# VaibhavKamat/Performance-Comparison-of-TensorFlow-PyTorch-and-their-Distributed-Counterparts

Hardware: AMD Instinct MI355X
Metric: resnet50_train_images_per_sec (higher is better)
Workload: dtype bf16; 1 GPU; model=resnet50, global_batch=256, per_gpu_batch=256, image_size=224, num_classes=1000, parallelism=dp1, impl=hip, optimizer=sgd_momentum, hipgraph=False, ddp_force=False, grad_allreduce_dtype=fp32, lr_warmup_steps=5

## Files before the change

### performance-comparison-of-tensorflow-pytorch-and-their-distributed-counterparts_amd/csrc/bnr_stream.h

```cpp
#pragma once
#include "igemm.h"

namespace pcmp {

inline Knob kn_bnr_stream("bnr_stream", 1);
inline Knob kn_bnr_stream_wgs("bnr_stream_wgs", 256);

template <int BN, int GK, bool FOLD, bool DUAL>
__global__ void __launch_bounds__(256, 2) bnr_stream_kernel(const IgemmParams p, int groups) {
  constexpr int BM = 32, NTHR = 256;
  constexpr int KB = GK / 64;
  constexpr int A_IMG = BM * GK * 2;
  constexpr int STAGE = A_IMG * (FOLD ? 2 : 1);
  constexpr int W_BYTES = BN * GK * 2;
  constexpr int CS = BN + 8;
  constexpr int C_BYTES = BM * CS * 4;
  constexpr int CPR = BN / 8;
  constexpr int NCH = BM * BN / 8 / NTHR;
  constexpr int RPP = NTHR / CPR;
  constexpr int NS = DUAL ? 3 : 2;
  constexpr int NWT = BN / 32;
  constexpr int NAI = A_IMG / 1024 / 4;
  constexpr int NWI = W_BYTES / 1024 / 4;
  constexpr int NEL = NCH * (DUAL ? 4 : 3);
  static_assert(NCH >= 1 && NAI >= 1 && NWI >= 1 && NWT <= 4, "bnr_stream tile");
  extern __shared__ __attribute__((aligned(16))) char smem[];
  char* sW = smem;
  char* sS = smem + W_BYTES;
  float* sC = reinterpret_cast<float*>(smem + W_BYTES + 2 * STAGE);
  float* sK = sC + BM * CS;

  const int tid = threadIdx.x, lane = tid & 63;
  const int wid = __builtin_amdgcn_readfirstlane(tid >> 6);
  const int ntn = p.gn / BN;
  const int lin = xcd_remap(blockIdx.x, gridDim.x);
  const int grp = lin / ntn, n0 = (lin - grp * ntn) * BN;
  const int npt = p.gm / BM;
  const int nmine = grp < npt ? (npt - 1 - grp) / groups + 1 : 0;

  const __amdgpu_buffer_rsrc_t rsA = make_rsrc(p.a, p.a_bytes);
  const __amdgpu_buffer_rsrc_t rsF = make_rsrc(FOLD ? p.fold_x : p.a, p.a_bytes);
  const __amdgpu_buffer_rsrc_t rsW = make_rsrc(p.b, p.b_bytes);
  const unsigned ebytes = (unsigned)((size_t)p.gm * p.gn * 2);
  const bool has_res = p.resid != nullptr;
  const unsigned rbytes = !has_res ? 0u : (p.resid_sub ? (unsigned)((size_t)p.N * p.rs_H2 * p.rs_W2 * p.gn * 2) : ebytes);
  const __amdgpu_buffer_rsrc_t rsR = make_rsrc(has_res ? (const void*)p.resid : (const void*)p.a, rbytes);
  const __amdgpu_buffer_rsrc_t rsX = make_rsrc(p.bn_x, ebytes);
  const __amdgpu_buffer_rsrc_t rsX2 = make_rsrc(DUAL ? p.bn_x2 : p.bn_x, DUAL ? ebytes : 0u);
  const bool has_mb = p.bn_mbits != nullptr;
  const __amdgpu_buffer_rsrc_t rsM = make_rsrc(has_mb ? (const void*)p.bn_mbits : (const void*)p.a,
                                               has_mb ? (unsigned)((size_t)p.gm * p.gn / 8) : 0u);

  const int lch = (lane & 7) ^ ((lane >> 3) & 7);
  int a_vo[NAI];
#pragma unroll
  for (int i = 0; i < NAI; ++i) {
    const int u = wid * NAI + i;
    const int row = (u & 3) * 8 + (lane >> 3);
    a_vo[i] = (row * GK + (u >> 2) * 64 + lch * 8) * 2;
  }
  const __amdgpu_buffer_rsrc_t rsZ = make_rsrc(p.a, 0u);
  auto issue_a = [&](int s, int pt, bool live) {
    char* dst = sS + s * STAGE;
    const int so = live ? pt * BM * GK * 2 : 0;
    const __amdgpu_buffer_rsrc_t ra = live ? rsA : rsZ, rf = live ? rsF : rsZ;
#pragma unroll
    for (int i = 0; i < NAI; ++i) {
      const int vo = a_vo[i];
      __builtin_amdgcn_raw_ptr_buffer_load_lds(ra, (__attribute__((address_space(3))) void*)(dst + (wid * NAI + i) * 1024),
                                               16, vo, so, 0, 0);
    }
    if constexpr (FOLD) {
#pragma unroll
      for (int i = 0; i < NAI; ++i) {
        const int vo = a_vo[i];
        __builtin_amdgcn_raw_ptr_buffer_load_lds(
            rf, (__attribute__((address_space(3))) void*)(dst + A_IMG + (wid * NAI + i) * 1024), 16, vo, so, 0, 0);
      }
    }
  };

  const int c8 = tid % CPR, r0 = tid / CPR;
  uint4 eR[2][NCH], eX[2][NCH], eX2[2][DUAL ? NCH : 1];
  unsigned eM[2][NCH];
  auto issue_e = [&](auto sel, int pt, bool live) {
    constexpr int E = decltype(sel)::value;
    if (!live) pt = 0;
    unsigned o[NCH], ro[NCH];
#pragma unroll
    for (int k = 0; k < NCH; ++k) {
      const int m = pt * BM + r0 + k * RPP;
      o[k] = (unsigned)m * (unsigned)p.gn + (unsigned)(n0 + c8 * 8);
      ro[k] = o[k] * 2u;
      if (p.resid_sub) {
        const unsigned n = fdiv((unsigned)m, p.fd_HW);
        const unsigned rem = (unsigned)m - n * (unsigned)(p.H * p.W);
        const unsigned hh = fdiv(rem, p.fd_W);
        const unsigned ww = rem - hh * (unsigned)p.W;
        ro[k] = ((hh | ww) & 1u) ? kOOB
                                 : (((n * (unsigned)p.rs_H2 + (hh >> 1)) * (unsigned)p.rs_W2 + (ww >> 1)) * (unsigned)p.gn +
                                    (unsigned)(n0 + c8 * 8)) * 2u;
      }
    }
#pragma unroll
    for (int k = 0; k < NCH; ++k) {
      if (!live) { o[k] = kOOB / 2u; ro[k] = kOOB; }
    }
#pragma unroll
    for (int k = 0; k < NCH; ++k) {
      eR[E][k] = bload16(rsR, ro[k]);
      eX[E][k] = bload16(rsX, o[k] * 2u);
      if constexpr (DUAL) eX2[E][k] = bload16(rsX2, o[k] * 2u);
      eM[E][k] = __builtin_amdgcn_raw_buffer_load_b32(rsM, (int)((o[k] >> 3) & ~3u), 0, 0);
    }
  };

  float ka[8], kb[8], ka2[DUAL ? 8 : 1], kb2[DUAL ? 8 : 1], msc[8], msh[8];
  const bool mfx = !has_mb;
#pragma unroll
  for (int e = 0; e < 8; ++e) {
    const int c = n0 + c8 * 8 + e;
    const float is = p.bn_istd[c];
    ka[e] = is;
    kb[e] = -p.bn_mean[c] * is;
    msc[e] = mfx ? p.bn_msc[c] : 0.f;
    msh[e] = mfx ? p.bn_msh[c] : 0.f;
    if constexpr (DUAL) {
      const float is2 = p.bn_istd2[c];
      ka2[e] = is2;
      kb2[e] = -p.bn_mean2[c] * is2;
    }
  }
  float sm[NS][8];
#pragma unroll
  for (int q = 0; q < NS; ++q)
#pragma unroll
    for (int e = 0; e < 8; ++e) sm[q][e] = 0.f;

  {
    int w_vo[NWI];
#pragma unroll
    for (int i = 0; i < NWI; ++i) {
      const int u = wid * NWI + i;
      const int row = (u % (BN / 8)) * 8 + (lane >> 3);
      w_vo[i] = ((n0 + row) * GK + (u / (BN / 8)) * 64 + lch * 8) * 2;
    }
#pragma unroll
    for (int i = 0; i < NWI; ++i) {
      const int vo = w_vo[i];
      __builtin_amdgcn_raw_ptr_buffer_load_lds(rsW, (__attribute__((address_space(3))) void*)(sW + (wid * NWI + i) * 1024),
                                               16, vo, 0, 0, 0);
    }
  }
  if constexpr (FOLD) {
    for (int i = tid; i < 3 * GK; i += NTHR) sK[i] = p.fold_coef[(i / GK) * p.K + (i % GK)];
  }
  const int pt0 = grp;
  issue_a(0, pt0, nmine > 0);
  issue_e(std::integral_constant<int, 0>{}, pt0, nmine > 0);
  wait_vm_b<0>();
  lds_sync_b();

  auto tile = [&](auto sel, int j) {
    constexpr int S = decltype(sel)::value;
    const int pt = pt0 + j * groups;
    if (j > 0) {
      wait_vm_b<NEL + NCH>();
      lds_sync_b();
    }
    char* sA = sS + S * STAGE;
    if constexpr (FOLD) {
#pragma unroll
      for (int i = 0; i < KB; ++i) {
        const int row = tid >> 3;
        const int kc = i * 64 + (((tid & 7) ^ (row & 7)) << 3);
        char* gp = sA + i * (BM * 128) + tid * 16;
        const uint4 g = *reinterpret_cast<const uint4*>(gp);
        const uint4 x = *reinterpret_cast<const uint4*>(gp + A_IMG);
        float k1[8], k2[8], k3[8];
#pragma unroll
        for (int h = 0; h < 2; ++h) {
          const f32x4 a = *reinterpret_cast<const f32x4*>(sK + kc + 4 * h);
          const f32x4 b = *reinterpret_cast<const f32x4*>(sK + GK + kc + 4 * h);
          const f32x4 c = *reinterpret_cast<const f32x4*>(sK + 2 * GK + kc + 4 * h);
#pragma unroll
          for (int e = 0; e < 4; ++e) { k1[4 * h + e] = a[e]; k2[4 * h + e] = b[e]; k3[4 * h + e] = c[e]; }
        }
        *reinterpret_cast<uint4*>(gp) = fold_dz(g, x, k1, k2, k3, true);
      }
      lds_sync_b();
    }
    __builtin_amdgcn_sched_barrier(0);
    const bool more = j + 1 < nmine;
    issue_a(S ^ 1, pt + groups, more);
    __builtin_amdgcn_sched_barrier(0);
    issue_e(std::integral_constant<int, S ^ 1>{}, pt + groups, more);
    __builtin_amdgcn_sched_barrier(0);
    if (wid < NWT) {
      f32x16 acc;
#pragma unroll
      for (int r = 0; r < 16; ++r) acc[r] = 0.f;
#pragma unroll
      for (int ks = 0; ks < GK / 16; ++ks) {
        const int ch = ks * 2 + (lane >> 5);
        const int kb = ch >> 3, cc = ch & 7;
        const bf16x8 fa = *reinterpret_cast<const bf16x8*>(sA + kb * (BM * 128) + rr_off(lane & 31, cc));
        const bf16x8 fb = *reinterpret_cast<const bf16x8*>(sW + kb * (BN * 128) + rr_off(wid * 32 + (lane & 31), cc));
        acc = __builtin_amdgcn_mfma_f32_32x32x16_bf16(fa, fb, acc, 0, 0, 0);
      }
#pragma unroll
      for (int r = 0; r < 16; ++r)
        sC[(8 * (r >> 2) + 4 * (lane >> 5) + (r & 3)) * CS + wid * 32 + (lane & 31)] = acc[r];
    }
    lds_sync_b();
    __bf16* out = reinterpret_cast<__bf16*>(p.out);
    const int mshift = ((n0 + c8 * 8) >> 3 & 3) * 8;
#pragma unroll
    for (int k = 0; k < NCH; ++k) {
      const int row = r0 + k * RPP;
      const f32x4 a0 = *reinterpret_cast<const f32x4*>(sC + row * CS + c8 * 8);
      const f32x4 a1 = *reinterpret_cast<const f32x4*>(sC + row * CS + c8 * 8 + 4);
      const float av[8] = {a0[0], a0[1], a0[2], a0[3], a1[0], a1[1], a1[2], a1[3]};
      const unsigned rw[4] = {eR[S][k].x, eR[S][k].y, eR[S][k].z, eR[S][k].w};
      const unsigned xw[4] = {eX[S][k].x, eX[S][k].y, eX[S][k].z, eX[S][k].w};
      unsigned ov[4];
#pragma unroll
      for (int q = 0; q < 4; ++q) {
        const float x0 = av[2 * q] + __uint_as_float(rw[q] << 16);
        const float x1 = av[2 * q + 1] + __uint_as_float(rw[q] & 0xffff0000u);
        unsigned u = f2bf2(x0, x1);
        const float xa = __uint_as_float(xw[q] << 16), xb = __uint_as_float(xw[q] & 0xffff0000u);
        const float z0 = fmaf(xa, msc[2 * q], msh[2 * q]);
        const float z1 = fmaf(xb, msc[2 * q + 1], msh[2 * q + 1]);
        const unsigned kz = (z0 > 0.f ? 0x0000ffffu : 0u) | (z1 > 0.f ? 0xffff0000u : 0u);
        const unsigned bits = eM[S][k] >> (mshift + 2 * q);
        const unsigned kbits = ((bits & 1u) ? 0x0000ffffu : 0u) | ((bits & 2u) ? 0xffff0000u : 0u);
        u &= mfx ? kz : kbits;
        const float g0 = __uint_as_float(u << 16), g1 = __uint_as_float(u & 0xffff0000u);
        sm[0][2 * q] += g0;
        sm[0][2 * q + 1] += g1;
        sm[1][2 * q] += g0 * fmaf(xa, ka[2 * q], kb[2 * q]);
        sm[1][2 * q + 1] += g1 * fmaf(xb, ka[2 * q + 1], kb[2 * q + 1]);
        if constexpr (DUAL) {
          const unsigned x2w = q == 0 ? eX2[S][k].x : q == 1 ? eX2[S][k].y : q == 2 ? eX2[S][k].z : eX2[S][k].w;
          sm[2][2 * q] += g0 * fmaf(__uint_as_float(x2w << 16), ka2[2 * q], kb2[2 * q]);
          sm[2][2 * q + 1] += g1 * fmaf(__uint_as_float(x2w & 0xffff0000u), ka2[2 * q + 1], kb2[2 * q + 1]);
        }
        ov[q] = u;
      }
      const size_t o = (size_t)(pt * BM + row) * p.gn + n0 + c8 * 8;
      *reinterpret_cast<uint4*>(out + o) = uint4{ov[0], ov[1], ov[2], ov[3]};
    }
  };
  int j = 0;
  for (; j + 1 < nmine; j += 2) {
    tile(std::integral_constant<int, 0>{}, j);
    tile(std::integral_constant<int, 1>{}, j + 1);
  }
  if (j < nmine) tile(std::integral_constant<int, 0>{}, j);

  __syncthreads();
  float* red = reinterpret_cast<float*>(sS);
#pragma unroll
  for (int q = 0; q < NS; ++q) {
    *reinterpret_cast<f32x4*>(red + (r0 * NS + q) * BN + c8 * 8) = f32x4{sm[q][0], sm[q][1], sm[q][2], sm[q][3]};
    *reinterpret_cast<f32x4*>(red + (r0 * NS + q) * BN + c8 * 8 + 4) = f32x4{sm[q][4], sm[q][5], sm[q][6], sm[q][7]};
  }
  __syncthreads();
  for (int i = tid; i < NS * BN; i += NTHR) {
    const int q = i / BN, c = i - q * BN;
    float t = 0.f;
    for (int r = 0; r < RPP; ++r) t += red[(r * NS + q) * BN + c];
    float* st = p.stats + (size_t)grp * 2 * p.gn;
    if (q == 0) {
      st[n0 + c] = t;
      if constexpr (DUAL) p.stats2[(size_t)grp * 2 * p.gn + n0 + c] = t;
    } else if (q == 1) {
      st[p.gn + n0 + c] = t;
    } else {
      p.stats2[(size_t)grp * 2 * p.gn + p.gn + n0 + c] = t;
    }
  }
}

static int bnr_stream_bn(const IgemmParams& p) { return p.gn == 64 ? 64 : 128; }

static bool use_bnr_stream(const IgemmParams& p) {
  if (!kn_bnr_stream.get() || !p.bn_x || p.R != 1 || p.S != 1 || p.stride != 1 || p.pad != 0) return false;
  if (!(p.gk == 64 || p.gk == 128 || p.gk == 256) || p.gn % bnr_stream_bn(p) || p.gm % 32) return false;
  if (!p.bn_mbits && !(p.bn_msc && !p.bn_mask)) return false;
  if (p.relu) return false;
  if ((p.fold_x ? 2 : 1) * p.gk >= p.gn) return false;
  return (int64_t)p.gm * p.gn * 2 < (1ll << 31) && (int64_t)p.gm * p.gk * 2 < (1ll << 31);
}

static int bnr_stream_groups(const IgemmParams& p) {
  const int ntn = p.gn / bnr_stream_bn(p);
  const int npt = p.gm / 32;
  return std::max(1, std::min(npt, std::max(1, kn_bnr_stream_wgs.get() / ntn)));
}

template <int BN, int GK, bool FOLD, bool DUAL>
static void launch_bnr_stream_cfg(IgemmParams& p, hipStream_t st) {
  constexpr int BM = 32;
  const int ntn = p.gn / BN;
  const int groups = bnr_stream_groups(p);
  TORCH_CHECK(p.stats && p.stats_cap >= groups && (!DUAL || p.stats2), "bnr_stream: partial-stats buffers");
  constexpr size_t stage = (size_t)BM * GK * 2 * (FOLD ? 2 : 1);
  constexpr size_t red = (size_t)(256 / (BN / 8)) * (DUAL ? 3 : 2) * BN * 4;
  constexpr size_t body = 2 * stage + (size_t)BM * (BN + 8) * 4 + (FOLD ? 3 * GK * 4 : 0);
  constexpr size_t smem = (size_t)BN * GK * 2 + std::max(body, red);
  static_assert(smem <= 160 * 1024, "bnr_stream: LDS");
  launch_lds<bnr_stream_kernel<BN, GK, FOLD, DUAL>>(dim3(groups * ntn), dim3(256), smem, st, p, groups);
}

static void launch_bnr_stream(IgemmParams& p, hipStream_t st) {
  const bool fold = p.fold_x != nullptr, dual = p.bn_x2 != nullptr;
  const int BN = bnr_stream_bn(p);
#define PCMP_BNRS(B, G)                                                                      \
  do {                                                                                      \
    if (fold) {                                                                             \
      if (dual) launch_bnr_stream_cfg<B, G, true, true>(p, st);                             \
      else launch_bnr_stream_cfg<B, G, true, false>(p, st);                                 \
    } else {                                                                                \
      if (dual) launch_bnr_stream_cfg<B, G, false, true>(p, st);                            \
      else launch_bnr_stream_cfg<B, G, false, false>(p, st);                                \
    }                                                                                       \
  } while (0)
  if (BN == 64) {
    if (p.gk == 64) PCMP_BNRS(64, 64); else if (p.gk == 128) PCMP_BNRS(64, 128); else PCMP_BNRS(64, 256);
  } else {
    if (p.gk == 64) PCMP_BNRS(128, 64); else if (p.gk == 128) PCMP_BNRS(128, 128); else PCMP_BNRS(128, 256);
  }
#undef PCMP_BNRS
}

}

namespace pcmp {

inline Knob kn_fwd_stream("fwd_stream", 1);
inline Knob kn_fwd_stream_wgs("fwd_stream_wgs", 512);

template <int BN, int GK, bool FOLD>
__global__ void __launch_bounds__(256, 2) fwd_stream_kernel(const IgemmParams p, int groups) {
  constexpr int BM = 32, NTHR = 256;
  constexpr int KB = GK / 64;
  constexpr int A_IMG = BM * GK * 2;
  constexpr int STAGE = A_IMG;
  constexpr int W_BYTES = BN * GK * 2;
  constexpr int CS = BN + 8;
  constexpr int CPR = BN / 8;
  constexpr int NCH = BM * BN / 8 / NTHR;
  constexpr int RPP = NTHR / CPR;
  constexpr int NWT = BN / 32;
  constexpr int TPW = NWT > 4 ? NWT / 4 : 1;
  constexpr int NAI = A_IMG / 1024 / 4;
  constexpr int NWI = W_BYTES / 1024 / 4;
  static_assert(NCH >= 1 && NAI >= 1 && NWI >= 1 && (NWT <= 4 || NWT % 4 == 0), "fwd_stream tile");
  extern __shared__ __attribute__((aligned(16))) char smem[];
  char* sW = smem;
  char* sS = smem + W_BYTES;
  float* sC = reinterpret_cast<float*>(smem + W_BYTES + 2 * STAGE);
  float* sK = sC + BM * CS;

  const int tid = threadIdx.x, lane = tid & 63;
  const int wid = __builtin_amdgcn_readfirstlane(tid >> 6);
  const int ntn = p.gn / BN;
  const int lin = xcd_remap(blockIdx.x, gridDim.x);
  const int grp = lin / ntn, n0 = (lin - grp * ntn) * BN;
  const int npt = p.gm / BM;
  const int nmine = grp < npt ? (npt - 1 - grp) / groups + 1 : 0;

  const __amdgpu_buffer_rsrc_t rsA = make_rsrc(p.a, p.a_bytes);
  const __amdgpu_buffer_rsrc_t rsW = make_rsrc(p.b, p.b_bytes);
  const __amdgpu_buffer_rsrc_t rsZ = make_rsrc(p.a, 0u);
  const int lch = (lane & 7) ^ ((lane >> 3) & 7);
  int a_vo[NAI];
#pragma unroll
  for (int i = 0; i < NAI; ++i) {
    const int u = wid * NAI + i;
    const int row = (u & 3) * 8 + (lane >> 3);
    a_vo[i] = (row * GK + (u >> 2) * 64 + lch * 8) * 2;
  }
  auto issue_a = [&](int s, int pt, bool live) {
    char* dst = sS + s * STAGE;
    const int so = live ? pt * BM * GK * 2 : 0;
    const __amdgpu_buffer_rsrc_t ra = live ? rsA : rsZ;
#pragma unroll
    for (int i = 0; i < NAI; ++i) {
      const int vo = a_vo[i];
      __builtin_amdgcn_raw_ptr_buffer_load_lds(ra, (__attribute__((address_space(3))) void*)(dst + (wid * NAI + i) * 1024),
                                               16, vo, so, 0, 0);
    }
  };
  {
    int w_vo[NWI];
#pragma unroll
    for (int i = 0; i < NWI; ++i) {
      const int u = wid * NWI + i;
      const int row = (u % (BN / 8)) * 8 + (lane >> 3);
      w_vo[i] = ((n0 + row) * GK + (u / (BN / 8)) * 64 + lch * 8) * 2;
    }
#pragma unroll
    for (int i = 0; i < NWI; ++i) {
      const int vo = w_vo[i];
      __builtin_amdgcn_raw_ptr_buffer_load_lds(rsW, (__attribute__((address_space(3))) void*)(sW + (wid * NWI + i) * 1024),
                                               16, vo, 0, 0, 0);
    }
  }
  if constexpr (FOLD) {
    for (int i = tid; i < 2 * GK; i += NTHR) sK[i] = i < GK ? p.act_sc[i] : p.act_sh[i - GK];
  }
  const int c8 = tid % CPR, r0 = tid / CPR;
  float sm[2][8];
#pragma unroll
  for (int q = 0; q < 2; ++q)
#pragma unroll
    for (int e = 0; e < 8; ++e) sm[q][e] = 0.f;
  const int pt0 = grp;
  issue_a(0, pt0, nmine > 0);
  wait_vm_b<0>();
  lds_sync_b();

  auto tile = [&](auto sel, int j) {
    constexpr int S = decltype(sel)::value;
    const int pt = pt0 + j * groups;
    if (j > 0) {
      wait_vm_b<NCH>();
      lds_sync_b();
    }
    char* sA = sS + S * STAGE;
    if constexpr (FOLD) {
#pragma unroll
      for (int i = 0; i < KB; ++i) {
        const int row = tid >> 3;
        const int kc = i * 64 + (((tid & 7) ^ (row & 7)) << 3);
        char* zp = sA + i * (BM * 128) + tid * 16;
        float a[8], b[8];
#pragma unroll
        for (int h = 0; h < 2; ++h) {
          const f32x4 u = *reinterpret_cast<const f32x4*>(sK + kc + 4 * h);
          const f32x4 v = *reinterpret_cast<const f32x4*>(sK + GK + kc + 4 * h);
#pragma unroll
          for (int e = 0; e < 4; ++e) { a[4 * h + e] = u[e]; b[4 * h + e] = v[e]; }
        }
        *reinterpret_cast<uint4*>(zp) = fold_act(*reinterpret_cast<const uint4*>(zp), a, b, true);
      }
      lds_sync_b();
    }
    __builtin_amdgcn_sched_barrier(0);
    issue_a(S ^ 1, pt + groups, j + 1 < nmine);
    __builtin_amdgcn_sched_barrier(0);
    if (wid < NWT) {
#pragma unroll
      for (int tt = 0; tt < TPW; ++tt) {
        const int ct = wid + 4 * tt;
        f32x16 acc;
#pragma unroll
        for (int r = 0; r < 16; ++r) acc[r] = 0.f;
#pragma unroll
        for (int ks = 0; ks < GK / 16; ++ks) {
          const int ch = ks * 2 + (lane >> 5);
          const int kb = ch >> 3, cc = ch & 7;
          const bf16x8 fa = *reinterpret_cast<const bf16x8*>(sA + kb * (BM * 128) + rr_off(lane & 31, cc));
          const bf16x8 fb = *reinterpret_cast<const bf16x8*>(sW + kb * (BN * 128) + rr_off(ct * 32 + (lane & 31), cc));
          acc = __builtin_amdgcn_mfma_f32_32x32x16_bf16(fa, fb, acc, 0, 0, 0);
        }
#pragma unroll
        for (int r = 0; r < 16; ++r)
          sC[(8 * (r >> 2) + 4 * (lane >> 5) + (r & 3)) * CS + ct * 32 + (lane & 31)] = acc[r];
      }
    }
    lds_sync_b();
    __bf16* out = reinterpret_cast<__bf16*>(p.out);
#pragma unroll
    for (int k = 0; k < NCH; ++k) {
      const int row = r0 + k * RPP;
      const f32x4 a0 = *reinterpret_cast<const f32x4*>(sC + row * CS + c8 * 8);
      const f32x4 a1 = *reinterpret_cast<const f32x4*>(sC + row * CS + c8 * 8 + 4);
      const float av[8] = {a0[0], a0[1], a0[2], a0[3], a1[0], a1[1], a1[2], a1[3]};
      unsigned ov[4];
#pragma unroll
      for (int q = 0; q < 4; ++q) {
        const unsigned u = f2bf2(av[2 * q], av[2 * q + 1]);
        const float y0 = __uint_as_float(u << 16), y1 = __uint_as_float(u & 0xffff0000u);
        sm[0][2 * q] += y0;
        sm[0][2 * q + 1] += y1;
        sm[1][2 * q] += y0 * y0;
        sm[1][2 * q + 1] += y1 * y1;
        ov[q] = u;
      }
      const size_t o = (size_t)(pt * BM + row) * p.gn + n0 + c8 * 8;
      *reinterpret_cast<uint4*>(out + o) = uint4{ov[0], ov[1], ov[2], ov[3]};
    }
  };
  int j = 0;
  for (; j + 1 < nmine; j += 2) {
    tile(std::integral_constant<int, 0>{}, j);
    tile(std::integral_constant<int, 1>{}, j + 1);
  }
  if (j < nmine) tile(std::integral_constant<int, 0>{}, j);

  __syncthreads();
  float* red = reinterpret_cast<float*>(sS);
#pragma unroll
  for (int q = 0; q < 2; ++q) {
    *reinterpret_cast<f32x4*>(red + (r0 * 2 + q) * BN + c8 * 8) = f32x4{sm[q][0], sm[q][1], sm[q][2], sm[q][3]};
    *reinterpret_cast<f32x4*>(red + (r0 * 2 + q) * BN + c8 * 8 + 4) = f32x4{sm[q][4], sm[q][5], sm[q][6], sm[q][7]};
  }
  __syncthreads();
  for (int i = tid; i < 2 * BN; i += NTHR) {
    const int q = i / BN, c = i - q * BN;
    float t = 0.f;
    for (int r = 0; r < RPP; ++r) t += red[(r * 2 + q) * BN + c];
    p.stats[(size_t)grp * 2 * p.gn + q * p.gn + n0 + c] = t;
  }
}

static bool use_fwd_stream(const IgemmParams& p) {
  if (!kn_fwd_stream.get() || p.bias || p.resid || p.relu) return false;
  if (p.R != 1 || p.S != 1 || p.stride != 1 || p.pad != 0) return false;
  if (!(p.gk == 64 || p.gk == 128) || p.gk >= p.gn || p.gn % 128 || p.gm % 32) return false;
  return (int64_t)p.gm * p.gn * 2 < (1ll << 31);
}
static int fwd_stream_bn(const IgemmParams& p) { return (p.gk == 64 && p.gn % 256 == 0) ? 256 : 128; }
static int fwd_stream_groups(const IgemmParams& p) {
  const int ntn = p.gn / fwd_stream_bn(p);
  return std::max(1, std::min(p.gm / 32, std::max(1, kn_fwd_stream_wgs.get() / ntn)));
}

template <int BN, int GK, bool FOLD>
static void launch_fwd_stream_cfg(IgemmParams& p, hipStream_t st) {
  constexpr int BM = 32;
  const int ntn = p.gn / BN;
  const int groups = fwd_stream_groups(p);
  TORCH_CHECK(p.stats && p.stats_cap >= groups, "fwd_stream: partial-stats buffer");
  constexpr size_t body = (size_t)2 * BM * GK * 2 + (size_t)BM * (BN + 8) * 4 + (FOLD ? 2 * GK * 4 : 0);
  constexpr size_t red = (size_t)(256 / (BN / 8)) * 2 * BN * 4;
  constexpr size_t smem = (size_t)BN * GK * 2 + std::max(body, red);
  static_assert(smem <= 160 * 1024, "fwd_stream: LDS");
  launch_lds<fwd_stream_kernel<BN, GK, FOLD>>(dim3(groups * ntn), dim3(256), smem, st, p, groups);
}

static void launch_fwd_stream(IgemmParams& p, hipStream_t st) {
  const bool fold = p.act_sc != nullptr;
  if (fwd_stream_bn(p) == 256) {
    if (fold) launch_fwd_stream_cfg<256, 64, true>(p, st); else launch_fwd_stream_cfg<256, 64, false>(p, st);
  } else if (p.gk == 64) {
    if (fold) launch_fwd_stream_cfg<128, 64, true>(p, st); else launch_fwd_stream_cfg<128, 64, false>(p, st);
  } else {
    if (fold) launch_fwd_stream_cfg<128, 128, true>(p, st); else launch_fwd_stream_cfg<128, 128, false>(p, st);
  }
}

}
```

Before: 14020 images/s.

## Extend fused BN-ReLU stream kernel to fold-wide shapes with aliased x/result LDS

Allows the bnr_stream fused GEMM+BN-backward path to handle folded cases where 2*gk >= gn (previously rejected), so these layers use the streaming kernel instead of a fallback. For BN=128, GK=128 with fold, the x image buffer is aliased with the fp32 result tile in LDS to cut shared memory, and the workgroup count is doubled for that case to raise occupancy. This adds layout complexity and a risk of LDS hazards between the x image and result tile across stages.

```diff
diff --git a/performance-comparison-of-tensorflow-pytorch-and-their-distributed-counterparts_amd/csrc/bnr_stream.h b/performance-comparison-of-tensorflow-pytorch-and-their-distributed-counterparts_amd/csrc/bnr_stream.h
--- a/performance-comparison-of-tensorflow-pytorch-and-their-distributed-counterparts_amd/csrc/bnr_stream.h
+++ b/performance-comparison-of-tensorflow-pytorch-and-their-distributed-counterparts_amd/csrc/bnr_stream.h
@@ -5,6 +5,8 @@
 
 inline Knob kn_bnr_stream("bnr_stream", 1);
 inline Knob kn_bnr_stream_wgs("bnr_stream_wgs", 256);
+
+constexpr bool bnr_stream_xalias(int bn, int gk, bool fold) { return fold && bn == 128 && gk == 128; }
 
 template <int BN, int GK, bool FOLD, bool DUAL>
 __global__ void __launch_bounds__(256, 2) bnr_stream_kernel(const IgemmParams p, int groups) {
@@ -24,11 +26,16 @@
   constexpr int NWI = W_BYTES / 1024 / 4;
   constexpr int NEL = NCH * (DUAL ? 4 : 3);
   static_assert(NCH >= 1 && NAI >= 1 && NWI >= 1 && NWT <= 4, "bnr_stream tile");
+  constexpr bool XALIAS = bnr_stream_xalias(BN, GK, FOLD);
+  static_assert(!XALIAS || C_BYTES > A_IMG, "bnr_stream: result tile over an x image");
   extern __shared__ __attribute__((aligned(16))) char smem[];
   char* sW = smem;
   char* sS = smem + W_BYTES;
+  char* sXB = sS + 2 * A_IMG;
   float* sC = reinterpret_cast<float*>(smem + W_BYTES + 2 * STAGE);
-  float* sK = sC + BM * CS;
+  float* sK = XALIAS ? reinterpret_cast<float*>(sXB + C_BYTES + A_IMG) : sC + BM * CS;
+  auto img_g = [&](int s) { return sS + s * (XALIAS ? A_IMG : STAGE); };
+  auto img_x = [&](int s) { return XALIAS ? sXB + s * C_BYTES : sS + s * STAGE + A_IMG; };
 
   const int tid = threadIdx.x, lane = tid & 63;
   const int wid = __builtin_amdgcn_readfirstlane(tid >> 6);
@@ -61,7 +68,7 @@
   }
   const __amdgpu_buffer_rsrc_t rsZ = make_rsrc(p.a, 0u);
   auto issue_a = [&](int s, int pt, bool live) {
-    char* dst = sS + s * STAGE;
+    char* dst = img_g(s);
     const int so = live ? pt * BM * GK * 2 : 0;
     const __amdgpu_buffer_rsrc_t ra = live ? rsA : rsZ, rf = live ? rsF : rsZ;
 #pragma unroll
@@ -71,11 +78,12 @@
                                                16, vo, so, 0, 0);
     }
     if constexpr (FOLD) {
+      char* dstx = img_x(s);
 #pragma unroll
       for (int i = 0; i < NAI; ++i) {
         const int vo = a_vo[i];
         __builtin_amdgcn_raw_ptr_buffer_load_lds(
-            rf, (__attribute__((address_space(3))) void*)(dst + A_IMG + (wid * NAI + i) * 1024), 16, vo, so, 0, 0);
+            rf, (__attribute__((address_space(3))) void*)(dstx + (wid * NAI + i) * 1024), 16, vo, so, 0, 0);
       }
     }
   };
@@ -168,15 +176,17 @@
       wait_vm_b<NEL + NCH>();
       lds_sync_b();
     }
-    char* sA = sS + S * STAGE;
+    char* sA = img_g(S);
+    float* sCt = XALIAS ? reinterpret_cast<float*>(sXB + S * A_IMG) : sC;
     if constexpr (FOLD) {
+      const char* sX = img_x(S);
 #pragma unroll
       for (int i = 0; i < KB; ++i) {
         const int row = tid >> 3;
         const int kc = i * 64 + (((tid & 7) ^ (row & 7)) << 3);
         char* gp = sA + i * (BM * 128) + tid * 16;
         const uint4 g = *reinterpret_cast<const uint4*>(gp);
-        const uint4 x = *reinterpret_cast<const uint4*>(gp + A_IMG);
+        const uint4 x = *reinterpret_cast<const uint4*>(sX + i * (BM * 128) + tid * 16);
         float k1[8], k2[8], k3[8];
 #pragma unroll
         for (int h = 0; h < 2; ++h) {
@@ -210,7 +220,7 @@
       }
 #pragma unroll
       for (int r = 0; r < 16; ++r)
-        sC[(8 * (r >> 2) + 4 * (lane >> 5) + (r & 3)) * CS + wid * 32 + (lane & 31)] = acc[r];
+        sCt[(8 * (r >> 2) + 4 * (lane >> 5) + (r & 3)) * CS + wid * 32 + (lane & 31)] = acc[r];
     }
     lds_sync_b();
     __bf16* out = reinterpret_cast<__bf16*>(p.out);
@@ -218,8 +228,8 @@
 #pragma unroll
     for (int k = 0; k < NCH; ++k) {
       const int row = r0 + k * RPP;
-      const f32x4 a0 = *reinterpret_cast<const f32x4*>(sC + row * CS + c8 * 8);
-      const f32x4 a1 = *reinterpret_cast<const f32x4*>(sC + row * CS + c8 * 8 + 4);
+      const f32x4 a0 = *reinterpret_cast<const f32x4*>(sCt + row * CS + c8 * 8);
+      const f32x4 a1 = *reinterpret_cast<const f32x4*>(sCt + row * CS + c8 * 8 + 4);
       const float av[8] = {a0[0], a0[1], a0[2], a0[3], a1[0], a1[1], a1[2], a1[3]};
       const unsigned rw[4] = {eR[S][k].x, eR[S][k].y, eR[S][k].z, eR[S][k].w};
       const unsigned xw[4] = {eX[S][k].x, eX[S][k].y, eX[S][k].z, eX[S][k].w};
@@ -283,21 +293,32 @@
   }
 }
 
-static int bnr_stream_bn(const IgemmParams& p) { return p.gn == 64 ? 64 : 128; }
+inline Knob kn_bnr_stream_foldwide("bnr_stream_foldwide", 1);
+
+static bool bnr_stream_is_foldwide(const IgemmParams& p) {
+  return p.fold_x && p.gk <= 128 && p.gk < p.gn && 2 * p.gk >= p.gn;
+}
+
+static int bnr_stream_bn(const IgemmParams& p) {
+  if (p.gn == 64) return 64;
+  return bnr_stream_is_foldwide(p) && kn_bnr_stream_foldwide.get() == 2 ? 64 : 128;
+}
 
 static bool use_bnr_stream(const IgemmParams& p) {
   if (!kn_bnr_stream.get() || !p.bn_x || p.R != 1 || p.S != 1 || p.stride != 1 || p.pad != 0) return false;
   if (!(p.gk == 64 || p.gk == 128 || p.gk == 256) || p.gn % bnr_stream_bn(p) || p.gm % 32) return false;
   if (!p.bn_mbits && !(p.bn_msc && !p.bn_mask)) return false;
   if (p.relu) return false;
-  if ((p.fold_x ? 2 : 1) * p.gk >= p.gn) return false;
+  if ((p.fold_x ? 2 : 1) * p.gk >= p.gn && !(kn_bnr_stream_foldwide.get() && bnr_stream_is_foldwide(p))) return false;
   return (int64_t)p.gm * p.gn * 2 < (1ll << 31) && (int64_t)p.gm * p.gk * 2 < (1ll << 31);
 }
 
 static int bnr_stream_groups(const IgemmParams& p) {
-  const int ntn = p.gn / bnr_stream_bn(p);
+  const int bn = bnr_stream_bn(p);
+  const int ntn = p.gn / bn;
   const int npt = p.gm / 32;
-  return std::max(1, std::min(npt, std::max(1, kn_bnr_stream_wgs.get() / ntn)));
+  const int per_cu = kn_bnr_stream_foldwide.get() == 1 && bnr_stream_is_foldwide(p) && bn == 128 && !p.bn_x2 ? 2 : 1;
+  return std::max(1, std::min(npt, std::max(1, per_cu * kn_bnr_stream_wgs.get() / ntn)));
 }
 
 template <int BN, int GK, bool FOLD, bool DUAL>
@@ -308,7 +329,8 @@
   TORCH_CHECK(p.stats && p.stats_cap >= groups && (!DUAL || p.stats2), "bnr_stream: partial-stats buffers");
   constexpr size_t stage = (size_t)BM * GK * 2 * (FOLD ? 2 : 1);
   constexpr size_t red = (size_t)(256 / (BN / 8)) * (DUAL ? 3 : 2) * BN * 4;
-  constexpr size_t body = 2 * stage + (size_t)BM * (BN + 8) * 4 + (FOLD ? 3 * GK * 4 : 0);
+  constexpr size_t body = 2 * stage + (size_t)BM * (BN + 8) * 4 + (FOLD ? 3 * GK * 4 : 0) -
+                          (bnr_stream_xalias(BN, GK, FOLD) ? (size_t)BM * GK * 2 : 0);
   constexpr size_t smem = (size_t)BN * GK * 2 + std::max(body, red);
   static_assert(smem <= 160 * 1024, "bnr_stream: LDS");
   launch_lds<bnr_stream_kernel<BN, GK, FOLD, DUAL>>(dim3(groups * ntn), dim3(256), smem, st, p, groups);
```

After: 14070 images/s, median of 6. About the same (+0.4%).
